# blue-yonder/tsfresh

Hardware: NVIDIA H100
Metric: series/sec extract_features ComprehensiveFCParameters (higher is better)
Workload: dtype f64

## Files before the change

### tsfresh_b200/csrc/k_la.cu

```cuda
#include <algorithm>

#include "tsfx_common.cuh"
#include "tsfx_kernels.h"
#include "tsfx_math.cuh"

namespace tsfx {

__host__ __device__ inline int adf_maxlag(int n) {
    int m = (int)ceil(12.0 * sqrt(sqrt((double)n / 100.0)));
    int cap = n / 2 - 2;
    return m < cap ? m : cap;
}

__device__ __forceinline__ void lag_gram(const double* seq, const double* lev, int t0, int T, int M, double* P, int ldp,
                                         double* C, double* Lv, int lane) {
    for (int d = lane; d <= M; d += 32) {
        double s = 0.0, c = 0.0, l = 0.0;
        for (int t = t0; t < T; ++t) {
            const double v = seq[t - d];
            s = fma(seq[t], v, s);
            c += v;
            if (lev) l = fma(lev[t], v, l);
        }
        C[d] = c;
        if (lev) Lv[d] = l;
        P[d * ldp + 0] = s;
        for (int i = 0; i + 1 + d <= M; ++i) {
            s += seq[t0 - i - 1] * seq[t0 - i - 1 - d] - seq[T - 1 - i] * seq[T - 1 - i - d];
            P[(i + 1 + d) * ldp + (i + 1)] = s;
        }
    }
    __syncwarp();
}

__device__ __forceinline__ int warp_cholesky(double* G, int q, int lda, int lane) {
    for (int j = 0; j < q; ++j) {
        double s = 0.0;
        for (int k = lane; k < j; k += 32) { double v = G[j * lda + k]; s = fma(v, v, s); }
        double d = G[j * lda + j] - wsum(s);
        if (!(d > 0.0)) return j;
        d = sqrt(d);
        __syncwarp();
        if (lane == 0) G[j * lda + j] = d;
        for (int i = j + 1 + lane; i < q; i += 32) {
            double t = G[i * lda + j];
            for (int k = 0; k < j; ++k) t = fma(-G[i * lda + k], G[j * lda + k], t);
            G[i * lda + j] = t / d;
        }
        __syncwarp();
    }
    return q;
}
__device__ __forceinline__ void warp_forward(const double* L, int q, int lda, double* b, int lane) {
    for (int k = 0; k < q; ++k) {
        double zk = b[k] / L[k * lda + k];
        __syncwarp();
        if (lane == 0) b[k] = zk;
        for (int i = k + 1 + lane; i < q; i += 32) b[i] = fma(-L[i * lda + k], zk, b[i]);
        __syncwarp();
    }
}
__device__ __forceinline__ void warp_backward(const double* L, int q, int lda, double* b, int lane) {
    for (int i = q - 1; i >= 0; --i) {
        double xi = b[i] / L[i * lda + i];
        __syncwarp();
        if (lane == 0) b[i] = xi;
        for (int k = lane; k < i; k += 32) b[k] = fma(-L[i * lda + k], xi, b[k]);
        __syncwarp();
    }
}

template <int WPC, bool GS>
__global__ void __launch_bounds__(WPC * 32) k_la(LaArgs A, int pmax) {
    extern __shared__ __align__(16) unsigned char smem_raw[];
    const int lane = threadIdx.x & 31, warp = threadIdx.x >> 5;
    unsigned char* base = warp_region<GS>(smem_raw, A.gscratch, A.bytes_per_warp, WPC, warp);
    double* xc = reinterpret_cast<double*>(base);
    double* dx = xc + A.npad;
    double* G = dx + A.npad;
    double* bvec = G + pmax * pmax;
    double* res = bvec + pmax;
    double* Pm = res + 8;
    double* Cv = Pm + pmax * pmax;
    double* Lv = Cv + pmax;
    float* xs = reinterpret_cast<float*>(Lv + pmax);
    const int64_t warps_total = (int64_t)gridDim.x * WPC;

    for (int64_t s = (int64_t)blockIdx.x * WPC + warp; s < A.R.n_series; s += warps_total) {
        const int n = load_series(A.R, s, xs, lane);
        const Moments M = moments(xs, n, xc, lane);
        for (int i = lane; i + 1 < n; i += 32) dx[i] = (double)xs[i + 1] - (double)xs[i];
        __syncwarp();
        double* orow = A.out + (size_t)s * A.ncols;
        int ar_k = -1; bool ar_ok = false;
        int adf_mode = -1;

        for (int j = 0; j < A.nd; ++j) {
            const Desc d = A.descs[j];
            double r = dnan();
            if (d.calc == TSFX_AR_COEFFICIENT) {
                const int k = d.i1, p = d.i0;
                if (k != ar_k) {
                    ar_k = k;
                    const int rows = n - k;
                    ar_ok = (k < n) && (rows >= k + 1);
                    if (ar_ok) {
                        const int q = k + 1;
                        lag_gram(xc, nullptr, k, n, k, Pm, pmax, Cv, nullptr, lane);
                        for (int e = lane; e < q * q; e += 32) {
                            const int a = e / q, c = e - a * q;
                            if (c > a) continue;
                            G[a * q + c] = (a == 0) ? (double)rows : (c == 0 ? Cv[a] : Pm[a * pmax + c]);
                        }
                        for (int a = lane; a < q; a += 32) bvec[a] = (a == 0) ? Cv[0] : Pm[a * pmax + 0];
                        __syncwarp();
                        int good = 0;
                        if (M.vmax == M.vmin) {
                            double cst = M.vmin, sc = cst / (1.0 + (double)k * cst * cst);
                            for (int a = lane; a < q; a += 32) bvec[a] = (a == 0) ? sc : sc * cst;
                            good = 2;
                        } else if (warp_cholesky(G, q, q, lane) == q) {
                            warp_forward(G, q, q, bvec, lane);
                            warp_backward(G, q, q, bvec, lane);
                            double sphi = 0.0;
                            for (int a = 1 + lane; a < q; a += 32) sphi += bvec[a];
                            sphi = wsum(sphi);
                            if (lane == 0) bvec[0] = bvec[0] + M.mean * (1.0 - sphi);
                            good = 1;
                        }
                        __syncwarp();
                        if (!good) { ar_ok = true; for (int a = lane; a <= k; a += 32) bvec[a] = dnan(); __syncwarp(); }
                    }
                }
                if (p > k) r = dnan();
                else if (!ar_ok) r = (p < k) ? dnan() : 0.0;
                else r = bvec[p];
            } else if (d.calc == TSFX_AUGMENTED_DICKEY_FULLER) {
                if (adf_mode != d.i0) {
                    adf_mode = d.i0;
                    __syncwarp();
                    double stat = dnan(), pval = dnan(), ulag = dnan();
                    const int M0 = adf_maxlag(n);
                    if (M.vmax != M.vmin && M0 >= 0) {
                        const int nd_ = n - 1;
                        int used = M0;
                        if (adf_mode != TSFX_AUTOLAG_NONE) {
                            const int p = M0 + 2, t0 = M0, nobs = nd_ - M0;
                            double* yy = res + 7;
                            lag_gram(dx, xc, t0, nd_, M0, Pm, pmax, Cv, Lv, lane);
                            {
                                double l1 = 0.0, l2 = 0.0;
                                for (int t = t0 + lane; t < nd_; t += 32) { double v = xc[t]; l1 += v; l2 = fma(v, v, l2); }
                                l1 = wsum(l1); l2 = wsum(l2);
                                for (int e = lane; e < p * p; e += 32) {
                                    const int a = e / p, c = e - a * p;
                                    if (c > a) continue;
                                    double v;
                                    if (a == 0) v = (double)nobs;
                                    else if (a == 1) v = (c == 0) ? l1 : l2;
                                    else v = (c == 0) ? Cv[a - 1] : (c == 1 ? Lv[a - 1] : Pm[(a - 1) * pmax + (c - 1)]);
                                    G[a * p + c] = v;
                                }
                                for (int a = lane; a < p; a += 32) bvec[a] = (a == 0) ? Cv[0] : (a == 1 ? Lv[0] : Pm[(a - 1) * pmax + 0]);
                                if (lane == 0) *yy = Pm[0];
                                __syncwarp();
                            }
                            int best_q = 2;
                            {
                                const int okq = warp_cholesky(G, p, p, lane);
                                double ssr = *yy;
                                double ssr_a = 0.0, ssr_b = 0.0;
                                const double dnobs = (double)nobs;
                                for (int i = 0; i < okq; ++i) {
                                    double z = bvec[i] / G[i * p + i];
                                    __syncwarp();
                                    for (int r2 = i + 1 + lane; r2 < okq; r2 += 32) bvec[r2] = fma(-G[r2 * p + i], z, bvec[r2]);
                                    __syncwarp();
                                    ssr -= z * z;
                                    if ((i & 31) == lane) { if (i < 32) ssr_a = ssr; else ssr_b = ssr; }
                                }
                                double ic_a = 0.0, ic_b = 0.0;
#pragma unroll
                                for (int c = 0; c < 2; ++c) {
                                    const int q = c * 32 + lane + 1;
                                    if (q >= 2 && q <= okq) {
                                        const double sq = c ? ssr_b : ssr_a;
                                        const double llf = -dnobs / 2.0 * log(2.0 * 3.14159265358979323846) -
                                                           dnobs / 2.0 * log(sq / dnobs) - dnobs / 2.0;
                                        const double pen = (adf_mode == TSFX_AUTOLAG_AIC) ? 2.0 * (double)q : log(dnobs) * (double)q;
                                        const double ic = -2.0 * llf + pen;
                                        if (c) ic_b = ic; else ic_a = ic;
                                    }
                                }
                                double best_ic = 0.0;
                                bool have = false;
                                for (int q = 2; q <= okq; ++q) {
                                    const double ic = __shfl_sync(FULL, (q > 32) ? ic_b : ic_a, (q - 1) & 31);
                                    if (!have || ic < best_ic) { have = true; best_ic = ic; best_q = q; }
                                }
                            }
                            best_q = __shfl_sync(FULL, best_q, 0);
                            used = best_q - 2;
                            __syncwarp();
                        }
                        const int q = used + 2, t0 = used, nobs = nd_ - used;
                        double* yy = res + 7;
                        lag_gram(dx, xc, t0, nd_, used, Pm, pmax, Cv, Lv, lane);
                        {
                            double l1 = 0.0, l2 = 0.0;
                            for (int t = t0 + lane; t < nd_; t += 32) { double v = xc[t]; l1 += v; l2 = fma(v, v, l2); }
                            l1 = wsum(l1); l2 = wsum(l2);
                            for (int e = lane; e < q * q; e += 32) {
                                const int a = e / q, c = e - a * q;
                                if (c > a) continue;
                                double v;
                                if (a == 0) v = (double)nobs;
                                else if (a < q - 1) v = (c == 0) ? Cv[a] : Pm[a * pmax + c];
                                else v = (c == 0) ? l1 : (c == q - 1 ? l2 : Lv[c]);
                                G[a * q + c] = v;
                            }
                            for (int a = lane; a < q; a += 32) bvec[a] = (a == 0) ? Cv[0] : (a < q - 1 ? Pm[a * pmax + 0] : Lv[0]);
                            if (lane == 0) *yy = Pm[0];
                            __syncwarp();
                        }
                        if (warp_cholesky(G, q, q, lane) == q) {
                            warp_forward(G, q, q, bvec, lane);
                            double ssr = 0.0;
                            for (int i = lane; i < q; i += 32) ssr = fma(bvec[i], bvec[i], ssr);
                            ssr = *yy - wsum(ssr);
                            double s2 = ssr / (double)(nobs - q);
                            stat = bvec[q - 1] / sqrt(s2);
                            pval = m_mackinnon_p_c(stat);
                            ulag = (double)used;
                        }
                        __syncwarp();
                        if (lane == 0) { res[0] = stat; res[1] = pval; res[2] = ulag; }
                    } else if (lane == 0) { res[0] = stat; res[1] = pval; res[2] = ulag; }
                    __syncwarp();
                }
                r = (d.attr >= 0 && d.attr <= 2) ? res[d.attr] : dnan();
            }
            if (lane == 0) orow[d.col] = r;
        }
        __syncwarp();
    }
}

cudaError_t launch_la(const LaArgs& A0, int max_len, cudaStream_t st, int sm_count, const char** variant) {
    static const char* const names[6] = TSFX_GEOM_NAMES("la");
    LaArgs A = A0;
    A.npad = (max_len + 3) & ~3;
    if (adf_maxlag(max_len) + 2 > 64) return cudaErrorInvalidConfiguration;
    int pmax = std::max(adf_maxlag(max_len) + 2, A.nscr + 1);
    pmax = (pmax + 1) & ~1;
    size_t per = (size_t)A.npad * 16 + (size_t)pmax * pmax * 16 + (size_t)pmax * 24 + 64 + (size_t)A.npad * 4;
    per = (per + 15) & ~(size_t)15;
    A.bytes_per_warp = (int)per;
    Geometry G;
    if (!plan_geometry(per, 100 * 1024, 8, A.R.n_series, sm_count, A.gscratch, A.gscratch_bytes, &G)) return cudaErrorInvalidConfiguration;
    A.gscratch = G.gscratch;
    *variant = geom_variant(names, G);
    TSFX_DISPATCH(k_la, G, st, A, pmax)
    return cudaGetLastError();
}

}
```

### tsfresh_b200/csrc/tsfx_api.cu

```cuda
#include <algorithm>
#include <cmath>
#include <cstdio>
#include <cstdlib>
#include <cstring>
#include <condition_variable>
#include <functional>
#include <map>
#include <mutex>
#include <new>
#include <string>
#include <thread>
#include <unordered_map>
#include <vector>

#include "tsfx_common.cuh"
#include "tsfx_kernels.h"
#include "tsfx_csr.h"
#include "tsfx_impute.h"
#include "tsfx_select.h"

using namespace tsfx;

static std::string g_create_error;

// ... 660 lines not shown
            case G_SORTED: {
                SortedArgs A;
                A.R = R; A.gscratch = gs_base; A.gscratch_bytes = slice; A.descs = P->dev[g]; A.nd = (int)P->host[g].size(); A.out = d_out; A.ncols = g_ncols;
                A.nscr = even(4 * (P->friedrich_r + 2) + 16);
                A.nfin = P->sorted_nfin;
                A.ncq = 0;
                {
                    double pl = -1.0, ph = -1.0;
                    for (const Desc& q : P->host[g])
                        if (q.calc == TSFX_CHANGE_QUANTILES && !(q.p0 == pl && q.p1 == ph)) { ++A.ncq; pl = q.p0; ph = q.p1; }
                }
                e = launch_sorted(A, max_len, gs, ctx->sm_count, &variant);
                break;
            }
            case G_SPECTRAL: {
                SpectralArgs A;
                A.R = R; A.gscratch = gs_base; A.gscratch_bytes = slice; A.descs = P->dev[g]; A.nd = (int)P->host[g].size(); A.out = d_out; A.ncols = g_ncols;
                A.twiddle = ctx->d_tw; A.tw_n = ctx->tw_n;
                A.tables = P->d_tables; A.table_off = P->d_toff; A.table_half = P->d_thalf;
                A.need_fft = P->need_fft; A.need_welch = P->need_welch;
                A.max_hist = P->fourier_bins;
                A.nfft = P->spectral_nfft;
                e = launch_spectral(A, max_len, gs, ctx->sm_count, &variant);
                break;
            }
            case G_LA: {
                LaArgs A;
                A.R = R; A.gscratch = gs_base; A.gscratch_bytes = slice; A.descs = P->dev[g]; A.nd = (int)P->host[g].size(); A.out = d_out; A.ncols = g_ncols;
                A.nscr = P->max_ar_k;
                e = launch_la(A, max_len, gs, ctx->sm_count, &variant);
                break;
            }
            case G_ENTROPY: {
                EntropyArgs A;
                A.R = R; A.gscratch = gs_base; A.gscratch_bytes = slice; A.descs = P->dev[g]; A.nd = (int)P->host[g].size(); A.out = d_out; A.ncols = g_ncols;
                e = launch_entropy(A, max_len, gs, ctx->sm_count, &variant);
                break;
            }
            case G_SEQ: {
                SeqArgs A;
                A.R = R; A.gscratch = gs_base; A.gscratch_bytes = slice; A.descs = P->dev[g]; A.nd = (int)P->host[g].size(); A.out = d_out; A.ncols = g_ncols;
                A.nscr = (P->max_lz_bins > 0 ? 1 : 0) | (P->max_perm_dim > 0 ? 2 : 0) | (P->max_cwt_peaks_n << 8) |
                         (std::min(P->n_lz, 255) << 16) | (std::min(P->max_lz_bins, 255) << 24);
                e = launch_seq(A, max_len, gs, ctx->sm_count, &variant);
                break;
            }
            case G_PEAKS: {
                SeqArgs A;
                A.R = R; A.gscratch = gs_base; A.gscratch_bytes = slice; A.descs = P->dev[g]; A.nd = (int)P->host[g].size(); A.out = d_out; A.ncols = g_ncols;
                A.nscr = (P->max_cwt_peaks_n << 8);
                A.ricker = ctx->d_ricker;
                e = launch_peaks(A, max_len, gs, ctx->sm_count, &variant);
                break;
            }
        }
        if (e == cudaErrorInvalidConfiguration) return too_long(kGroupNames[g]);
        if (e != cudaSuccess) return fail(ctx, TSFX_E_CUDA, std::string("launch ") + kGroupNames[g] + ": " + cudaGetErrorString(e));
        ctx->launches += 1;
        ctx->kernels[ctx->n_kernels++] = variant;
        if (timing) { CK(cudaEventRecord(ctx->ev[g][1], ctx->stream)); ctx->ev_used[g] = true; }
    }
    if (nstreams > 1)
        for (int i = 0; i < nstreams - 1; ++i) {
            CK(cudaEventRecord(ctx->ev_join[i], ctx->s_side[i]));
            CK(cudaStreamWaitEvent(ctx->stream, ctx->ev_join[i], 0));
        }
    if (!direct) {
        if (timing) { CK(cudaEventRecord(ctx->ev[G_COUNT][0], ctx->stream)); }
        AssembleArgs A;
        A.stage = (const double*)ctx->stage.p; A.out = d_final; A.n_series = R.n_series; A.ncols = P->ncols; A.ld = ld;
        if (ld != P->ncols && !ctx->peer_out.empty()) return fail(ctx, TSFX_E_UNSUPPORTED, "peer placement of a strided matrix");
        A.n_groups = G_COUNT;
        for (int g = 0; g <= G_COUNT; ++g) A.cum[g] = P->cum[g];
        A.final_col = P->d_final_col;
        A.n_extra = 0;
        A.out_mc = nullptr;
        int64_t peer_off = -1;
        if (!ctx->peer_out.empty()) {
            const uint64_t self = ctx->peer_out[ctx->peer_self];
            if ((uint64_t)d_final < self) return fail(ctx, TSFX_E_INVALID, "out is not inside the matrix registered with tsfx_set_peer_outputs");
            peer_off = (int64_t)((uint64_t)d_final - self);
            if (ctx->peer_mode == TSFX_PEER_MULTICAST) A.out_mc = (double*)(ctx->peer_mc + (uint64_t)peer_off);
            else if (ctx->peer_mode == TSFX_PEER_STORE)
                for (size_t p = 0; p < ctx->peer_out.size(); ++p)
                    if ((int)p != ctx->peer_self) A.extra[A.n_extra++] = (double*)(ctx->peer_out[p] + (uint64_t)peer_off);
        }
        cudaError_t e = launch_assemble(A, ctx->stream, ctx->sm_count);
        if (e != cudaSuccess) return fail(ctx, TSFX_E_CUDA, std::string("launch assemble: ") + cudaGetErrorString(e));
        ctx->launches += 1;
        if (timing) { CK(cudaEventRecord(ctx->ev[G_COUNT][1], ctx->stream)); ctx->ev_used[G_COUNT] = true; }
        if (peer_off >= 0 && ctx->peer_mode == TSFX_PEER_COPY) {
            const size_t bytes = (size_t)R.n_series * P->ncols * sizeof(double);
            CK(cudaEventRecord(ctx->ev_peer, ctx->stream));
            CK(cudaStreamWaitEvent(ctx->s_peer, ctx->ev_peer, 0));
            const size_t np = ctx->peer_out.size();
            for (size_t k = 1; k < np; ++k) {
                const size_t p = ((size_t)ctx->peer_self + k) % np;
                CK(cudaMemcpyAsync((void*)(ctx->peer_out[p] + (uint64_t)peer_off), d_final, bytes, cudaMemcpyDeviceToDevice, ctx->s_peer));
            }
        }
    }
    return TSFX_OK;
}

static int impute_after_extract(tsfx_ctx* ctx, double* d_out, int64_t rows, int cols);
static int nan_error(tsfx_ctx* ctx);

static int check_args(tsfx_ctx* ctx, const tsfx_plan* plan, const void* values, const void* out, int64_t n_series) {
    if (!ctx) return TSFX_E_INVALID;
    if (!plan || plan->ctx != ctx) return fail(ctx, TSFX_E_INVALID, "plan does not belong to this context");
    if (n_series < 0) return fail(ctx, TSFX_E_INVALID, "n_series < 0");
    if (n_series > 0 && (!values || !out)) return fail(ctx, TSFX_E_INVALID, "NULL values/out");
    return TSFX_OK;
}

extern "C" int tsfx_extract_csr(tsfx_ctx* ctx, const tsfx_plan* plan, const float* values, int64_t n_values,
                                const int64_t* begin, const int32_t* len, int64_t n_series, double* out,
                                uint32_t flags) {
    int rc = check_args(ctx, plan, values, out, n_series);
    if (rc) return rc;
    if (n_series == 0) return TSFX_OK;
    if (!begin || !len) return fail(ctx, TSFX_E_INVALID, "NULL begin/len");
    CK(cudaSetDevice(ctx->device));
    SeriesRef R;
    R.dense_len = 0;
    R.n_series = n_series;
    rc = take_times(ctx, plan, n_values, &R.times);
    if (rc) return rc;
    int max_len = 0;
    if (flags & TSFX_FLAG_DEVICE_PTRS) {
        R.values = values; R.begin = begin; R.len = len;
        if (ctx->max_len_hint > 0) max_len = ctx->max_len_hint;
        else {
            int rc2 = csr_max_len(ctx->csr, len, n_series, ctx->stream, &max_len);
            if (rc2) return fail(ctx, TSFX_E_CUDA, "max-length reduction failed");
        }
        rc = run_groups(ctx, plan, R, max_len, out, flags);
        if (!rc && (flags & TSFX_FLAG_IMPUTE)) rc = impute_after_extract(ctx, out, n_series, plan->ncols);
        return rc;
    }
    for (int64_t s = 0; s < n_series; ++s) {
        if (len[s] < 1 || begin[s] < 0 || begin[s] + len[s] > n_values)
            return fail(ctx, TSFX_E_INVALID, "series " + std::to_string(s) + " has an invalid (begin, len)");
        max_len = std::max(max_len, (int)len[s]);
    }
    size_t ob = (size_t)n_series * plan->ncols * sizeof(double);
    CK(ctx->values.reserve((size_t)n_values * sizeof(float) + 16));
    CK(ctx->begin.reserve((size_t)n_series * sizeof(int64_t)));
    CK(ctx->len.reserve((size_t)n_series * sizeof(int32_t)));
    CK(ctx->out.reserve(std::max<size_t>(ob, 8)));
    CK(cudaMemcpyAsync(ctx->values.p, values, (size_t)n_values * sizeof(float), cudaMemcpyHostToDevice, ctx->stream));
    CK(cudaMemcpyAsync(ctx->begin.p, begin, (size_t)n_series * sizeof(int64_t), cudaMemcpyHostToDevice, ctx->stream));
    CK(cudaMemcpyAsync(ctx->len.p, len, (size_t)n_series * sizeof(int32_t), cudaMemcpyHostToDevice, ctx->stream));
    R.values = (const float*)ctx->values.p; R.begin = (const int64_t*)ctx->begin.p; R.len = (const int32_t*)ctx->len.p;
    const bool check_nan = !(flags & TSFX_FLAG_NO_NAN_CHECK);
    if (check_nan) {
        CK(ctx->csr.init_info());
        CK(cudaMemsetAsync(ctx->csr.d_info, 0, sizeof(CsrInfo), ctx->stream));
        csr_check_nan(ctx->csr, R.values, n_values, ctx->stream);
        CK(cudaMemcpyAsync(ctx->csr.h_info, ctx->csr.d_info, sizeof(CsrInfo), cudaMemcpyDeviceToHost, ctx->stream));
    }
    rc = run_groups(ctx, plan, R, max_len, (double*)ctx->out.p, flags);
    if (rc) return rc;
    if (flags & TSFX_FLAG_IMPUTE) { rc = impute_after_extract(ctx, (double*)ctx->out.p, n_series, plan->ncols); if (rc) return rc; }
    CK(cudaMemcpyAsync(out, ctx->out.p, ob, cudaMemcpyDeviceToHost, ctx->stream));
    CK(cudaStreamSynchronize(ctx->stream));
    if (check_nan && ctx->csr.h_info->has_nan) return nan_error(ctx);
    return TSFX_OK;
}

extern "C" int tsfx_extract_dense(tsfx_ctx* ctx, const tsfx_plan* plan, const float* values, int64_t n_series,
                                  int32_t len, double* out, uint32_t flags) {
    int rc = check_args(ctx, plan, values, out, n_series);
    if (rc) return rc;
    if (n_series == 0) return TSFX_OK;
    if (len < 1) return fail(ctx, TSFX_E_INVALID, "len < 1");
    CK(cudaSetDevice(ctx->device));
    SeriesRef R;
    R.begin = nullptr; R.len = nullptr; R.dense_len = len; R.n_series = n_series;
    const int64_t* all_times = nullptr;
    rc = take_times(ctx, plan, n_series * (int64_t)len, &all_times);
    if (rc) return rc;
    R.times = all_times;
    if (flags & TSFX_FLAG_DEVICE_PTRS) {
        R.values = values;
        rc = run_groups(ctx, plan, R, len, out, flags);
        if (!rc && (flags & TSFX_FLAG_IMPUTE)) rc = impute_after_extract(ctx, out, n_series, plan->ncols);
        return rc;
    }
    const size_t ncols = (size_t)plan->ncols;
    const size_t vb = (size_t)n_series * len * sizeof(float), ob = (size_t)n_series * ncols * sizeof(double);
    CK(ctx->values.reserve(vb + 16));
    CK(ctx->out.reserve(std::max<size_t>(ob, 8)));
    int64_t block = std::max<int64_t>(16384, (n_series + 15) / 16);
    if (flags & TSFX_FLAG_TIMING) block = n_series;
    float* dv = (float*)ctx->values.p;
    double* dout = (double*)ctx->out.p;
    const bool check_nan = !(flags & TSFX_FLAG_NO_NAN_CHECK);
    if (check_nan) { CK(ctx->csr.init_info()); CK(cudaMemsetAsync(ctx->csr.d_info, 0, sizeof(CsrInfo), ctx->stream)); }
    int nb = 0;
    for (int64_t lo = 0; lo < n_series; lo += block, ++nb) {
        const int64_t cnt = std::min<int64_t>(block, n_series - lo);
        const int slot = nb & 1;
        CK(ctx->stager.h2d(dv + (size_t)lo * len, values + (size_t)lo * len, (size_t)cnt * len * sizeof(float), ctx->s_in));
        CK(cudaEventRecord(ctx->ev_in[slot], ctx->s_in));
        CK(cudaStreamWaitEvent(ctx->stream, ctx->ev_in[slot], 0));
        if (check_nan) csr_check_nan(ctx->csr, dv + (size_t)lo * len, cnt * len, ctx->stream);
        R.values = dv + (size_t)lo * len;
        R.times = all_times ? all_times + (size_t)lo * len : nullptr;
        R.n_series = cnt;
        rc = run_groups(ctx, plan, R, len, dout + (size_t)lo * ncols, flags);
        if (rc) return rc;
        if (flags & TSFX_FLAG_IMPUTE) continue;
        CK(cudaEventRecord(ctx->ev_done[slot], ctx->stream));
        CK(cudaStreamWaitEvent(ctx->s_out, ctx->ev_done[slot], 0));
        CK(cudaMemcpyAsync(out + (size_t)lo * ncols, dout + (size_t)lo * ncols, (size_t)cnt * ncols * sizeof(double),
                           cudaMemcpyDeviceToHost, ctx->s_out));
    }
    if (flags & TSFX_FLAG_IMPUTE) {
        rc = impute_after_extract(ctx, dout, n_series, plan->ncols);
        if (rc) return rc;
        CK(cudaMemcpyAsync(out, dout, ob, cudaMemcpyDeviceToHost, ctx->stream));
    }
    if (check_nan) CK(cudaMemcpyAsync(ctx->csr.h_info, ctx->csr.d_info, sizeof(CsrInfo), cudaMemcpyDeviceToHost, ctx->stream));
    CK(cudaStreamSynchronize(ctx->s_out));
    CK(cudaStreamSynchronize(ctx->stream));
    if (check_nan && ctx->csr.h_info->has_nan) return nan_error(ctx);
    return TSFX_OK;
}

static int impute_after_extract(tsfx_ctx* ctx, double* d_out, int64_t rows, int cols) {
    int n = 0;
    cudaError_t e = impute_device(ctx->imp, d_out, rows, cols, TSFX_IMPUTE_RANGE, false, nullptr, ctx->sm_count, ctx->stream, &n);
    if (e != cudaSuccess) return fail(ctx, TSFX_E_CUDA, std::string("impute: ") + cudaGetErrorString(e));
    ctx->launches += n;
    return TSFX_OK;
}

extern "C" int tsfx_impute(tsfx_ctx* ctx, double* matrix, int64_t n_rows, int32_t n_cols, int32_t mode, double* col_stats,
                           uint32_t flags) {
    if (!ctx) return TSFX_E_INVALID;
    if (n_rows < 0 || n_cols < 0 || mode < TSFX_IMPUTE_RANGE || mode > TSFX_IMPUTE_STATS)
        return fail(ctx, TSFX_E_INVALID, "tsfx_impute: bad arguments");
    if (n_rows == 0 || n_cols == 0) return TSFX_OK;
    if (!matrix) return fail(ctx, TSFX_E_INVALID, "tsfx_impute: NULL matrix");
    if ((mode == TSFX_IMPUTE_GIVEN || mode == TSFX_IMPUTE_STATS) && !col_stats)
        return fail(ctx, TSFX_E_INVALID, "tsfx_impute: col_stats is required for this mode");
    if (mode == TSFX_IMPUTE_GIVEN)
        for (int64_t i = 0; i < (int64_t)3 * n_cols; ++i)
            if (!std::isfinite(col_stats[i]))
                return fail(ctx, TSFX_E_INVALID, "tsfx_impute: non-finite replacement value");
    CK(cudaSetDevice(ctx->device));
    const size_t bytes = (size_t)n_rows * n_cols * sizeof(double);
    double* d_m = matrix;
    const bool host = !(flags & TSFX_FLAG_DEVICE_PTRS);
    if (host) {
        CK(ctx->out.reserve(bytes));
        d_m = (double*)ctx->out.p;
        CK(cudaMemcpyAsync(d_m, matrix, bytes, cudaMemcpyHostToDevice, ctx->stream));
    }
    int n = 0;
    cudaError_t e = impute_device(ctx->imp, d_m, n_rows, n_cols, mode, (flags & TSFX_FLAG_ALL_MEDIANS) != 0 || mode == TSFX_IMPUTE_STATS,
                                  col_stats, ctx->sm_count, ctx->stream, &n);
    if (e != cudaSuccess) return fail(ctx, TSFX_E_CUDA, std::string("impute: ") + cudaGetErrorString(e));
    ctx->launches = n;
    if (host) {
        if (mode != TSFX_IMPUTE_STATS) CK(cudaMemcpyAsync(matrix, d_m, bytes, cudaMemcpyDeviceToHost, ctx->stream));
        CK(cudaStreamSynchronize(ctx->stream));
    }
    return TSFX_OK;
}

extern "C" int tsfx_get_timings(tsfx_ctx* ctx, float* ms_out, const char** names_out, int32_t cap) {
    if (!ctx) return TSFX_E_INVALID;
    CK(cudaSetDevice(ctx->device));
    CK(cudaStreamSynchronize(ctx->stream));
    int k = 0;
    for (int g = 0; g < G_EVENTS && k < cap; ++g) {
        if (!ctx->ev_used[g]) continue;
        float ms = 0.f;
        CK(cudaEventElapsedTime(&ms, ctx->ev[g][0], ctx->ev[g][1]));
        if (ms_out) ms_out[k] = ms;
        if (names_out) names_out[k] = (g == G_BASIC && ctx->used_moments) ? "moments" : kGroupNames[g];
        ++k;
    }
    return k;
}

extern "C" int tsfx_last_launch_count(const tsfx_ctx* ctx) { return ctx ? ctx->launches : 0; }

extern "C" int tsfx_last_kernels(const tsfx_ctx* ctx, const char** names_out, int32_t cap) {
    if (!ctx || cap < 0 || (cap > 0 && !names_out)) return TSFX_E_INVALID;
    const int k = std::min<int>(ctx->n_kernels, cap);
    for (int i = 0; i < k; ++i) names_out[i] = ctx->kernels[i];
    return k;
}

#define TSFX_GEOM_LIST(GRP) GRP "/w8/shared", GRP "/w4/shared", GRP "/w2/shared", GRP "/w1/shared", GRP "/w4/global", GRP "/w1/global"
static const char* const kKernelVariants[] = {
    "moments/dense", "moments/general",
    "basic/w12/shared", "basic/w24/shared", TSFX_GEOM_LIST("basic"),
    "sorted/w12/shared", TSFX_GEOM_LIST("sorted"),
    TSFX_GEOM_LIST("spectral"), TSFX_GEOM_LIST("spectral/pow2"),
    TSFX_GEOM_LIST("la"),
    "entropy/rank-g1", "entropy/rank-g4", "entropy/rank-g16", TSFX_GEOM_LIST("entropy/tiles"), TSFX_GEOM_LIST("entropy/pairs"),
    "seq/small", TSFX_GEOM_LIST("seq/general"),
    "peaks/small", TSFX_GEOM_LIST("peaks/general"), "peaks/general/hybrid/w4/global", "peaks/general/hybrid/w1/global",
};
#undef TSFX_GEOM_LIST

extern "C" int tsfx_kernel_variants(const char** names_out, int32_t cap) {
    const int n = (int)(sizeof(kKernelVariants) / sizeof(kKernelVariants[0]));
    for (int i = 0; i < n && i < cap && names_out; ++i) names_out[i] = kKernelVariants[i];
    return n;
}

struct LongIn {
    const int64_t* ids;
    const void* keys;
    int is_f64;
    const float* values;
    int64_t n;
    bool device;
    const float* const* more = nullptr;
    int n_kinds = 1;
    const float* col(int k) const { return k == 0 ? values : more[k - 1]; }
};

static inline size_t kind_stride(int64_t n) { return ((size_t)n + 3) & ~(size_t)3; }

static int nan_error(tsfx_ctx* ctx) { return fail(ctx, TSFX_E_NAN, "the value column contains NaN"); }

static int stage_a(tsfx_ctx* ctx, const LongIn& in, int max_blocks, bool check_nan, CsrInfo* info, bool* streamed,
                   const int64_t** d_ids_out, const uint64_t** d_keys_out, const float** d_vals_out) {
    CsrWorkspace& W = ctx->csr;
    std::string msg;
    const int64_t n = in.n;
    const int64_t* d_ids = in.ids;
    const uint64_t* d_keys = (const uint64_t*)in.keys;
    const float* d_vals = in.values;
    if (!in.device) {
        CK(W.reserve(0, (size_t)n * 8));
        CK(W.reserve(2, (size_t)n * 4 + 16));
        if (in.keys) CK(W.reserve(1, (size_t)n * 8));
        CK(ctx->stager.h2d(W.ids(), in.ids, (size_t)n * 8, ctx->stream));
        d_ids = W.ids();
        d_keys = in.keys ? W.keys() : nullptr;
        d_vals = W.vals();
    }
    int rc = csr_ids_pass(W, d_ids, n, 16384, max_blocks, ctx->stream, &msg);
    if (rc) return fail(ctx, rc, msg);
    CK(cudaStreamSynchronize(ctx->stream));
    *info = *W.h_info;
    *streamed = false;
    if (!info->unsorted_ids) {
        W.d_values = const_cast<float*>(d_vals);
        if (!in.device) *streamed = true;
        else csr_check_rows(W, d_ids, d_keys, in.is_f64, d_vals, 0, n, check_nan, ctx->stream);
    }
    *d_ids_out = d_ids; *d_keys_out = d_keys; *d_vals_out = d_vals;
    return TSFX_OK;
}

static int stage_a_sort(tsfx_ctx* ctx, const LongIn& in, int max_blocks, bool check_nan, CsrInfo* info,
                        const int64_t* d_ids, const uint64_t* d_keys, const float* d_vals) {
    CsrWorkspace& W = ctx->csr;
    std::string msg;
    if (!in.device) {
        if (in.keys) CK(ctx->stager.h2d(W.keys(), in.keys, (size_t)in.n * 8, ctx->stream));
        CK(ctx->stager.h2d(W.vals(), in.values, (size_t)in.n * 4, ctx->stream));
    }
    int rc = csr_sort_pass(W, d_ids, d_keys, in.is_f64, d_vals, in.n, 16384, max_blocks, check_nan, ctx->stream, &msg);
    if (rc) return fail(ctx, rc, msg);
    CK(cudaStreamSynchronize(ctx->stream));
    *info = *W.h_info;
    return TSFX_OK;
}

extern "C" int tsfx_build_csr(tsfx_ctx* ctx, const int64_t* ids, const void* sort_keys, int32_t sort_key_is_f64,
                              const float* values, int64_t n_rows, int64_t* out_ids, int64_t* out_begin,
                              int32_t* out_len, float* sorted_values, int64_t out_capacity, int64_t* n_series_out) {
    if (!ctx) return TSFX_E_INVALID;
    if (n_rows < 0 || !n_series_out || (n_rows > 0 && (!ids || !values)))
        return fail(ctx, TSFX_E_INVALID, "tsfx_build_csr: bad arguments");
    CK(cudaSetDevice(ctx->device));
    *n_series_out = 0;
    if (n_rows == 0) return TSFX_OK;
    ctx->held_series = -1;
    LongIn in{ids, sort_keys, sort_key_is_f64, values, n_rows, false};
    CsrInfo info;
    bool streamed = false;
    const int64_t* d_ids; const uint64_t* d_keys; const float* d_vals;
    int rc = stage_a(ctx, in, 1, true, &info, &streamed, &d_ids, &d_keys, &d_vals);
    if (rc) return rc;
    CsrWorkspace& W = ctx->csr;
    bool need_sort = info.unsorted_ids != 0;
    if (!need_sort) {
        if (sort_keys) CK(ctx->stager.h2d(W.keys(), sort_keys, (size_t)n_rows * 8, ctx->stream));
        CK(ctx->stager.h2d(W.vals(), values, (size_t)n_rows * 4, ctx->stream));
        csr_check_rows(W, d_ids, d_keys, sort_key_is_f64, d_vals, 0, n_rows, true, ctx->stream);
        CK(cudaMemcpyAsync(W.h_info, W.d_info, sizeof(CsrInfo), cudaMemcpyDeviceToHost, ctx->stream));
        CK(cudaStreamSynchronize(ctx->stream));
        info = *W.h_info;
        need_sort = info.unsorted_keys != 0;
        if (need_sort) {
            LongIn dev{d_ids, d_keys, sort_key_is_f64, d_vals, n_rows, true};
            rc = stage_a_sort(ctx, dev, 1, true, &info, d_ids, d_keys, d_vals);
            if (rc) return rc;
        }
    } else {
        rc = stage_a_sort(ctx, in, 1, true, &info, d_ids, d_keys, d_vals);
        if (rc) return rc;
    }
    if (info.has_nan) return nan_error(ctx);
    const int64_t ns = info.n_series;
    ctx->held_series = ns;
    ctx->held_max_len = info.max_len;
    *n_series_out = ns;
    if (!out_ids && !out_begin && !out_len && !sorted_values) return TSFX_OK;
    if (ns > out_capacity) return fail(ctx, TSFX_E_INVALID, "out_capacity too small: " + std::to_string(ns) + " series");
    if (out_ids) CK(cudaMemcpyAsync(out_ids, W.d_uid, ns * sizeof(int64_t), cudaMemcpyDeviceToHost, ctx->stream));
    if (out_begin) CK(cudaMemcpyAsync(out_begin, W.d_begin, ns * sizeof(int64_t), cudaMemcpyDeviceToHost, ctx->stream));
    if (out_len) CK(cudaMemcpyAsync(out_len, W.d_len, ns * sizeof(int32_t), cudaMemcpyDeviceToHost, ctx->stream));
    if (sorted_values) CK(cudaMemcpyAsync(sorted_values, W.d_values, n_rows * sizeof(float), cudaMemcpyDeviceToHost, ctx->stream));
    CK(cudaStreamSynchronize(ctx->stream));
    return TSFX_OK;
}

#define TSFX_MAX_KINDS 64
struct KindSet {
    int n = 1;
    const tsfx_plan* plan[TSFX_MAX_KINDS];
    const float* dvals[TSFX_MAX_KINDS];
    int col0[TSFX_MAX_KINDS];
    int total_cols = 0;
};

static int run_blocks(tsfx_ctx* ctx, const KindSet& K, const CsrInfo& info, const LongIn* stream_in,
                      const int64_t* d_ids, const uint64_t* d_keys, bool check_rows, bool check_nan,
                      double* out, bool out_is_device, uint32_t flags, const int64_t* row_times = nullptr) {
    CsrWorkspace& W = ctx->csr;
    const size_t ncols = (size_t)K.total_cols;
    const int64_t ns = info.n_series;
    double* dout = out;
    if (!out_is_device) {
        CK(ctx->out.reserve(std::max<size_t>((size_t)ns * ncols * sizeof(double), 8)));
        dout = (double*)ctx->out.p;
    }
    const bool impute = (flags & TSFX_FLAG_IMPUTE) != 0;
    for (int b = 0; b < info.n_blocks; ++b) {
        const int64_t s0 = info.series_lo[b], s1 = info.series_lo[b + 1];
        const int64_t r0 = info.row_lo[b], r1 = info.row_lo[b + 1];
        const int slot = b & 1;
        if (stream_in) {
            if (stream_in->keys) CK(ctx->stager.h2d(W.keys() + r0, (const uint64_t*)stream_in->keys + r0, (size_t)(r1 - r0) * 8, ctx->s_in));
            for (int k = 0; k < K.n; ++k)
                CK(ctx->stager.h2d(const_cast<float*>(K.dvals[k]) + r0, stream_in->col(k) + r0, (size_t)(r1 - r0) * 4, ctx->s_in));
            CK(cudaEventRecord(ctx->ev_in[slot], ctx->s_in));
            CK(cudaStreamWaitEvent(ctx->stream, ctx->ev_in[slot], 0));
        }
        if (check_rows) {
            csr_check_rows(W, d_ids, d_keys, stream_in ? stream_in->is_f64 : 0, K.dvals[0], r0, r1, check_nan, ctx->stream);
            if (check_nan) for (int k = 1; k < K.n; ++k) csr_check_nan(W, K.dvals[k] + r0, r1 - r0, ctx->stream);
        }
        for (int k = 0; k < K.n; ++k) {
            if (K.plan[k]->ncols == 0) continue;
            SeriesRef R;
            R.values = K.dvals[k]; R.begin = W.d_begin + s0; R.len = W.d_len + s0; R.dense_len = 0; R.n_series = s1 - s0;
            R.times = row_times;
            int rc = run_groups(ctx, K.plan[k], R, info.max_len, dout + (size_t)s0 * ncols + K.col0[k], flags, K.total_cols);
            if (rc) return rc;
        }
        if (impute || out_is_device) continue;
        CK(cudaEventRecord(ctx->ev_done[slot], ctx->stream));
        CK(cudaStreamWaitEvent(ctx->s_out, ctx->ev_done[slot], 0));
        CK(cudaMemcpyAsync(out + (size_t)s0 * ncols, dout + (size_t)s0 * ncols, (size_t)(s1 - s0) * ncols * sizeof(double),
                           cudaMemcpyDeviceToHost, ctx->s_out));
    }
    if (impute) {
        int rc = impute_after_extract(ctx, dout, ns, K.total_cols);
        if (rc) return rc;
        if (!out_is_device) CK(cudaMemcpyAsync(out, dout, (size_t)ns * ncols * sizeof(double), cudaMemcpyDeviceToHost, ctx->stream));
    }
    return TSFX_OK;
}

static int extract_long_impl(tsfx_ctx* ctx, const tsfx_plan* const* plans, const LongIn& in, int64_t* out_ids, double* out,
                             int64_t out_capacity, int64_t** out_ids_alloc, double** out_alloc, int64_t* n_series_out,
                             uint32_t flags) {
    CsrWorkspace& W = ctx->csr;
    const tsfx_plan* plan = plans[0];
    KindSet K;
    K.n = in.n_kinds;
    if (K.n < 1 || K.n > TSFX_MAX_KINDS) return fail(ctx, TSFX_E_INVALID, "between 1 and 64 kinds per call");
    for (int k = 0; k < K.n; ++k) {
        if (!plans[k] || plans[k]->ctx != ctx) return fail(ctx, TSFX_E_INVALID, "plan does not belong to this context");
        K.plan[k] = plans[k];
        K.col0[k] = K.total_cols;
        K.total_cols += plans[k]->ncols;
    }
    for (int k = 0; k < K.n; ++k) if (plans[k]->need_times) plan = plans[k];
    const size_t kstride = kind_stride(in.n);
    if (K.n > 1 && !in.device) CK(ctx->kvals.reserve((size_t)(K.n - 1) * kstride * 4 + 16));
    const bool check_nan = !(flags & TSFX_FLAG_NO_NAN_CHECK);
    const int max_blocks = (flags & TSFX_FLAG_TIMING) ? 1 : 16;
    ctx->held_series = -1;
    const int64_t* times_in = nullptr;
    int rc = take_times(ctx, plan, in.n, &times_in);
    if (rc) return rc;
    CsrInfo info;
    bool streamed = false;
    const int64_t* d_ids; const uint64_t* d_keys; const float* d_vals;
    rc = stage_a(ctx, in, max_blocks, check_nan, &info, &streamed, &d_ids, &d_keys, &d_vals);
    if (rc) return rc;
    bool sorted = !info.unsorted_ids;
    bool extra_resident = in.device;
    auto extra_in = [&](int k) -> const float* {
        return in.device ? in.col(k) : (const float*)ctx->kvals.p + (size_t)(k - 1) * kstride;
    };
    if (sorted && in.device && check_nan)
        for (int k = 1; k < K.n; ++k) csr_check_nan(W, in.col(k), in.n, ctx->stream);
    for (int attempt = 0; attempt < 2; ++attempt) {
        if (!sorted) {
            rc = stage_a_sort(ctx, in, max_blocks, check_nan, &info, d_ids, d_keys, d_vals);
            if (rc) return rc;
            if (info.has_nan) return nan_error(ctx);
        }
        K.dvals[0] = W.d_values;
        if (K.n > 1) {
            if (W.d_perm) {
                CK(ctx->kvals_sorted.reserve((size_t)(K.n - 1) * kstride * 4 + 16));
                for (int k = 1; k < K.n; ++k) {
                    if (!extra_resident) CK(ctx->stager.h2d(const_cast<float*>(extra_in(k)), in.col(k), (size_t)in.n * 4, ctx->stream));
                    if (check_nan) csr_check_nan(W, extra_in(k), in.n, ctx->stream);
                    float* dst = (float*)ctx->kvals_sorted.p + (size_t)(k - 1) * kstride;
                    csr_gather_f32(W, extra_in(k), dst, in.n, ctx->stream);
                    K.dvals[k] = dst;
                }
                extra_resident = true;
            } else {
                for (int k = 1; k < K.n; ++k) K.dvals[k] = extra_in(k);
            }
        }
        const int64_t ns = info.n_series;
        *n_series_out = ns;
        const size_t ob = (size_t)ns * K.total_cols * sizeof(double);
        if (out_alloc) {
            if (!*out_alloc) {
                *out_alloc = (double*)ctx->pool.alloc(std::max<size_t>(ob, 8));
                *out_ids_alloc = (int64_t*)ctx->pool.alloc(std::max<size_t>((size_t)ns * 8, 8));
                if (!*out_alloc || !*out_ids_alloc) return fail(ctx, TSFX_E_NOMEM, "pinned host allocation failed");
            }
            out = *out_alloc;
            out_ids = *out_ids_alloc;
        } else if (ns > out_capacity) {
            return fail(ctx, TSFX_E_INVALID, "out_capacity too small: " + std::to_string(ns) + " series");
        }
        if (info.max_len < 1 && ns > 0) return fail(ctx, TSFX_E_INVALID, "empty series");
        const bool first_sorted_try = sorted && attempt == 0;
        const int64_t* row_times = times_in;
        if (times_in && W.d_perm) {
            CK(ctx->times_sorted.reserve((size_t)in.n * 8));
            csr_gather_i64(W, times_in, (int64_t*)ctx->times_sorted.p, in.n, ctx->stream);
            row_times = (const int64_t*)ctx->times_sorted.p;
        }
        rc = run_blocks(ctx, K, info, (first_sorted_try && streamed) ? &in : nullptr, d_ids, d_keys,
                        first_sorted_try && streamed, check_nan, out, in.device, flags, row_times);
        if (first_sorted_try && streamed) extra_resident = true;
        if (rc) return rc;
        if (out_ids) CK(cudaMemcpyAsync(out_ids, W.d_uid, (size_t)ns * sizeof(int64_t), in.device ? cudaMemcpyDeviceToDevice : cudaMemcpyDeviceToHost, ctx->stream));
        if (in.device && !first_sorted_try) break;
        const bool late_nan_flags = !first_sorted_try && K.n > 1 && check_nan;
        if (first_sorted_try || late_nan_flags) CK(cudaMemcpyAsync(W.h_info, W.d_info, sizeof(CsrInfo), cudaMemcpyDeviceToHost, ctx->stream));
        CK(cudaStreamSynchronize(ctx->s_out));
        CK(cudaStreamSynchronize(ctx->stream));
        if (late_nan_flags && W.h_info->has_nan) return nan_error(ctx);
        if (!first_sorted_try) break;
        if (W.h_info->has_nan) return nan_error(ctx);
        if (!W.h_info->unsorted_keys) break;
        sorted = false;
        if (!in.device) {
            LongIn dev{d_ids, d_keys, in.is_f64, d_vals, in.n, true};
            rc = stage_a_sort(ctx, dev, max_blocks, check_nan, &info, d_ids, d_keys, d_vals);
            if (rc) return rc;
            if (info.has_nan) return nan_error(ctx);
            sorted = true;
            streamed = false;
        }
    }
    ctx->held_series = info.n_series;
    ctx->held_max_len = info.max_len;
    return TSFX_OK;
}

extern "C" int tsfx_extract_long(tsfx_ctx* ctx, const tsfx_plan* plan, const int64_t* ids, const void* sort_keys,
                                 int32_t sort_key_is_f64, const float* values, int64_t n_rows, int64_t* out_ids,
                                 double* out, int64_t out_capacity, int64_t* n_series_out, uint32_t flags) {
    if (!ctx) return TSFX_E_INVALID;
    if (!plan || plan->ctx != ctx) return fail(ctx, TSFX_E_INVALID, "plan does not belong to this context");
    const bool reuse = (ids == nullptr && values == nullptr);
    if (n_rows < 0 || !n_series_out || (!reuse && n_rows > 0 && (!ids || !values)) || !out)
        return fail(ctx, TSFX_E_INVALID, "tsfx_extract_long: bad arguments");
    CK(cudaSetDevice(ctx->device));
    *n_series_out = 0;
    if (reuse) {
        if (flags & TSFX_FLAG_DEVICE_PTRS) return fail(ctx, TSFX_E_INVALID, "the held CSR is extracted into host buffers");
        if (ctx->held_series < 0) return fail(ctx, TSFX_E_INVALID, "tsfx_extract_long: no CSR is held by this context");
// ... 214 lines not shown
```

Measured before the change: 4.456 million.

## Add register-resident small-series linear-algebra kernel for AR and ADF features

Adds a specialized k_la_small kernel for series up to 256 points with few AR lags. Gram matrices are built with a warp reduce-scatter plus incremental edge corrections, and Cholesky factorization runs with rows held in registers using a refined approximate rsqrt. ADF lag selection reuses a single full factorization to derive SSR for every lag. This is meant to cut the shared/global scratch traffic and per-lag refactorization of the generic path, at the cost of more register pressure and subtle numeric differences.

```diff
diff --git a/tsfresh_b200/csrc/k_la.cu b/tsfresh_b200/csrc/k_la.cu
--- a/tsfresh_b200/csrc/k_la.cu
+++ b/tsfresh_b200/csrc/k_la.cu
@@ -246,8 +246,344 @@
     }
 }
 
+#define LA_SMALL_LEN 256
+#define LA_SMALL_KMAX 15
+#define LA_SMALL_P 19
+#define LA_SMALL_LD 19
+#define LA_SMALL_WPC 8
+#define LA_SMALL_CB (LA_SMALL_P + 64)
+
+__device__ __forceinline__ double rsqrt_pos(double d) {
+    double y;
+    asm("rsqrt.approx.ftz.f64 %0, %1;" : "=d"(y) : "d"(d));
+#pragma unroll
+    for (int it = 0; it < 2; ++it) y = fma(0.5 * y, fma(-d * y, y, 1.0), y);
+    return y;
+}
+
+template <int O>
+__device__ __forceinline__ void reduce_scatter_stage(double (&v)[32], int lane) {
+    const bool up = lane & O;
+#pragma unroll
+    for (int i = 0; i < O; ++i) {
+        const double lo = v[i], hi = v[i + O];
+        const double send = up ? lo : hi;
+        const double keep = up ? hi : lo;
+        v[i] = keep + __shfl_xor_sync(FULL, send, O);
+    }
+    if constexpr (O > 1) reduce_scatter_stage<O / 2>(v, lane);
+}
+__device__ __forceinline__ double reduce_scatter32(double (&v)[32], int lane) {
+    reduce_scatter_stage<16>(v, lane);
+    return v[0];
+}
+
+__device__ __forceinline__ double pick(const double (&g)[LA_SMALL_P], int i) {
+    double r = 0.0;
+#pragma unroll
+    for (int c = 0; c < LA_SMALL_P; ++c)
+        if (c == i) r = g[c];
+    return r;
+}
+
+__device__ __forceinline__ int chol_rows(double (&g)[LA_SMALL_P], int na, int nf, double& inv, double* cb, int lane) {
+    double* piv = cb;
+    int done = nf;
+    if (lane == 0) piv[0] = g[0];
+#pragma unroll
+    for (int j = 0; j < LA_SMALL_P - 1; ++j) {
+        if (j < done) {
+            __syncwarp();
+            const double d = piv[j];
+            if (!(d > 0.0)) {
+                done = j;
+            } else {
+                double* col = cb + LA_SMALL_P + 32 * (j & 1);
+                const double rinv = rsqrt_pos(d), r = d * rinv;
+                const double l = (lane == j) ? r : g[j] * rinv;
+                if (lane == j) inv = rinv;
+                if (lane >= j) g[j] = l;
+                col[lane] = l;
+                __syncwarp();
+#pragma unroll
+                for (int c = j + 1; c < LA_SMALL_P; ++c) {
+                    const double lc = col[c];
+                    g[c] = (lane > j) ? fma(-l, lc, g[c]) : (lane == j ? lc : g[c]);
+                }
+                if (j + 1 < LA_SMALL_P && lane == j + 1) piv[j + 1] = g[j + 1];
+            }
+        }
+    }
+    __syncwarp();
+    return done;
+}
+
+template <typename F>
+__device__ __forceinline__ void load_rows(double (&g)[LA_SMALL_P], const double* Gs, int na, F col, int lane) {
+    const double* row = Gs + (lane < na ? col(lane) : 0) * LA_SMALL_LD;
+#pragma unroll
+    for (int c = 0; c < LA_SMALL_P; ++c) g[c] = (c < na && lane < na) ? row[col(c)] : 0.0;
+}
+
+template <int NL>
+__device__ __forceinline__ void ar_sums(double (&v)[32], const double* xs, int n, int k, double mean, int lane) {
+#pragma unroll 1
+    for (int t = k + lane; t < n; t += 32) {
+        const double w = xs[t] - mean;
+        v[16] += w;
+#pragma unroll
+        for (int d = 0; d < NL; ++d) v[d] = fma(w, xs[max(t - d, 0)] - mean, v[d]);
+    }
+}
+
+__device__ __forceinline__ void ar_gram(const double* xs, int n, int k, double mean, double* Gs, int lane) {
+    double v[32];
+#pragma unroll
+    for (int i = 0; i < 32; ++i) v[i] = 0.0;
+    if (k <= 10) ar_sums<11>(v, xs, n, k, mean, lane);
+    else ar_sums<LA_SMALL_KMAX + 1>(v, xs, n, k, mean, lane);
+    const double tot = reduce_scatter32(v, lane);
+    const double c0 = __shfl_sync(FULL, tot, 16);
+    __syncwarp();
+    const int q = k + 1;
+    auto col = [&](int i) { return i == 0 ? q : i; };
+    auto xc = [&](int i) { return xs[i] - mean; };
+    if (lane <= k) {
+        const int d = lane;
+        double s = tot, c = c0;
+        Gs[col(d) * LA_SMALL_LD + col(0)] = s;
+        Gs[col(0) * LA_SMALL_LD + col(d)] = s;
+        for (int m = 0; m + 1 + d <= k; ++m) {
+            s += xc(k - m - 1) * xc(k - m - 1 - d) - xc(n - 1 - m) * xc(n - 1 - m - d);
+            Gs[col(m + 1 + d) * LA_SMALL_LD + col(m + 1)] = s;
+            Gs[col(m + 1) * LA_SMALL_LD + col(m + 1 + d)] = s;
+        }
+        for (int m = 0; m < d; ++m) c += xc(k - 1 - m) - xc(n - 1 - m);
+        Gs[col(d)] = c;
+        Gs[col(d) * LA_SMALL_LD] = c;
+    }
+    if (lane == 0) Gs[0] = (double)(n - k);
+    __syncwarp();
+}
+
+__device__ __forceinline__ void adf_gram(const double* xs, int n, int M0, double mean, double* Gs, int lane) {
+    const int nd = n - 1, t0 = M0, p = M0 + 2;
+    auto xd = [&](int i) { return xs[i]; };
+    auto dx = [&](int i) { return xd(i + 1) - xd(i); };
+    auto col = [&](int i) { return i == 0 ? p : i + 1; };
+    double sums[2];
+#pragma unroll
+    for (int pass = 0; pass < 2; ++pass) {
+        double v[32];
+#pragma unroll
+        for (int i = 0; i < 32; ++i) v[i] = 0.0;
+#pragma unroll 1
+        for (int t = t0 + lane; t < nd; t += 32) {
+            double hi = xd(t + 1), lo = xd(t);
+            const double y = hi - lo, lev = lo - mean;
+            const double w = pass ? lev : y;
+            if (!pass) { v[17] += lev; v[18] = fma(lev, lev, v[18]); }
+#pragma unroll
+            for (int d = 0; d <= 16; ++d) {
+                if (d > 0) { hi = lo; lo = xd(max(t - d, 0)); }
+                v[d] = fma(w, hi - lo, v[d]);
+            }
+        }
+        sums[pass] = reduce_scatter32(v, lane);
+    }
+    const double tot = sums[0], lv = sums[1];
+    const double l1 = __shfl_sync(FULL, tot, 17), l2 = __shfl_sync(FULL, tot, 18);
+    __syncwarp();
+    if (lane <= M0) {
+        const int d = lane;
+        double s = tot;
+        Gs[col(d) * LA_SMALL_LD + col(0)] = s;
+        Gs[col(0) * LA_SMALL_LD + col(d)] = s;
+        for (int m = 0; m + 1 + d <= M0; ++m) {
+            s += dx(t0 - m - 1) * dx(t0 - m - 1 - d) - dx(nd - 1 - m) * dx(nd - 1 - m - d);
+            Gs[col(m + 1 + d) * LA_SMALL_LD + col(m + 1)] = s;
+            Gs[col(m + 1) * LA_SMALL_LD + col(m + 1 + d)] = s;
+        }
+        const double c = xd(nd - d) - xd(t0 - d);
+        Gs[col(d)] = c;
+        Gs[col(d) * LA_SMALL_LD] = c;
+        Gs[LA_SMALL_LD + col(d)] = lv;
+        Gs[col(d) * LA_SMALL_LD + 1] = lv;
+    }
+    if (lane == 0) {
+        Gs[0] = (double)(nd - M0);
+        Gs[1] = Gs[LA_SMALL_LD] = l1;
+        Gs[LA_SMALL_LD + 1] = l2;
+    }
+    __syncwarp();
+}
+
+template <int WPC, int MINB>
+__global__ void __launch_bounds__(WPC * 32, MINB) k_la_small(LaArgs A) {
+    extern __shared__ __align__(16) unsigned char smem_raw[];
+    const int lane = threadIdx.x & 31, warp = threadIdx.x >> 5;
+    unsigned char* base = smem_raw + (size_t)warp * A.bytes_per_warp;
+    double* xs = reinterpret_cast<double*>(base);
+    double* Gs = xs + LA_SMALL_LEN;
+    double* cb = Gs + LA_SMALL_P * LA_SMALL_LD;
+    double* arb = cb + LA_SMALL_CB;
+
+    for (int64_t s = (int64_t)blockIdx.x * WPC + warp; s < A.R.n_series; s += (int64_t)gridDim.x * WPC) {
+        float* stage = reinterpret_cast<float*>(Gs);
+        const int n = load_series(A.R, s, stage, lane);
+        const Moments M = moments(stage, n, nullptr, lane);
+        for (int i = lane; i < n; i += 32) xs[i] = (double)stage[i];
+        __syncwarp();
+        const bool flat = M.vmax == M.vmin;
+        int ar_k = -1; bool ar_ok = false;
+        int adf_mode = -1; bool adf_gram_ok = false;
+
+        for (int j = 0; j < A.nd; ++j) {
+            const Desc d = A.descs[j];
+            double r = dnan();
+            if (d.calc == TSFX_AR_COEFFICIENT) {
+                const int k = d.i1, p = d.i0;
+                if (k != ar_k) {
+                    ar_k = k;
+                    const int rows = n - k;
+                    ar_ok = (k < n) && (rows >= k + 1);
+                    if (ar_ok) {
+                        const int q = k + 1;
+                        if (flat) {
+                            const double cst = M.vmin, sc = cst / (1.0 + (double)k * cst * cst);
+                            if (lane < q) arb[lane] = (lane == 0) ? sc : sc * cst;
+                        } else {
+                            ar_gram(xs, n, k, M.mean, Gs, lane);
+                            adf_gram_ok = false;
+                            double g[LA_SMALL_P], inv = 0.0;
+                            load_rows(g, Gs, q + 1, [](int i) { return i; }, lane);
+                            if (chol_rows(g, q + 1, q, inv, cb, lane) == q) {
+                                double b = pick(g, q);
+#pragma unroll
+                                for (int i = LA_SMALL_P - 2; i >= 0; --i) {
+                                    if (i < q) {
+                                        if (lane == i) arb[i] = b * inv;
+                                        __syncwarp();
+                                        if (lane < i) b = fma(-g[i], arb[i], b);
+                                    }
+                                }
+                                if (lane == 0) {
+                                    double sphi = 0.0;
+                                    for (int a = 1; a < q; ++a) sphi += arb[a];
+                                    arb[0] = arb[0] + M.mean * (1.0 - sphi);
+                                }
+                            } else if (lane < q) {
+                                arb[lane] = dnan();
+                            }
+                        }
+                        __syncwarp();
+                    }
+                }
+                if (p > k) r = dnan();
+                else if (!ar_ok) r = (p < k) ? dnan() : 0.0;
+                else r = arb[p];
+            } else if (d.calc == TSFX_AUGMENTED_DICKEY_FULLER) {
+                if (adf_mode != d.i0) {
+                    adf_mode = d.i0;
+                    double stat = dnan(), pval = dnan(), ulag = dnan();
+                    const int M0 = adf_maxlag(n);
+                    if (!flat && M0 >= 0) {
+                        const int nd_ = n - 1, p = M0 + 2;
+                        if (!adf_gram_ok) { adf_gram(xs, n, M0, M.mean, Gs, lane); adf_gram_ok = true; }
+                        int used = M0;
+                        if (adf_mode != TSFX_AUTOLAG_NONE) {
+                            double g[LA_SMALL_P], inv = 0.0;
+                            load_rows(g, Gs, p + 1, [](int i) { return i; }, lane);
+                            const int okq = chol_rows(g, p + 1, p, inv, cb, lane);
+                            if (lane == p) {
+#pragma unroll
+                                for (int c = 0; c < LA_SMALL_P - 1; ++c) cb[c] = g[c];
+                            }
+                            __syncwarp();
+                            const double dnobs = (double)(nd_ - M0);
+                            double ssr = Gs[p * LA_SMALL_LD + p], ssr_q = 0.0;
+                            for (int i = 0; i < okq; ++i) {
+                                const double z = cb[i];
+                                ssr -= z * z;
+                                if (lane == i) ssr_q = ssr;
+                            }
+                            double ic = 0.0;
+                            const int q = lane + 1;
+                            if (q >= 2 && q <= okq) {
+                                const double llf = -dnobs / 2.0 * log(2.0 * 3.14159265358979323846) -
+                                                   dnobs / 2.0 * log(ssr_q / dnobs) - dnobs / 2.0;
+                                const double pen = (adf_mode == TSFX_AUTOLAG_AIC) ? 2.0 * (double)q : log(dnobs) * (double)q;
+                                ic = -2.0 * llf + pen;
+                            }
+                            __syncwarp();
+                            cb[lane] = ic;
+                            __syncwarp();
+                            int best_q = 2;
+                            double best_ic = 0.0;
+                            bool have = false;
+                            for (int qq = 2; qq <= okq; ++qq) {
+                                const double icq = cb[qq - 1];
+                                if (!have || icq < best_ic) { have = true; best_ic = icq; best_q = qq; }
+                            }
+                            __syncwarp();
+                            used = best_q - 2;
+                        }
+                        const int q = used + 2, na = q + 1;
+                        auto fcol = [&](int f) { return f == 0 ? 0 : f <= used ? f + 1 : f == used + 1 ? 1 : p; };
+                        double g[LA_SMALL_P], inv = 0.0;
+                        load_rows(g, Gs, na, fcol, lane);
+                        for (int t = used; t < M0; ++t) {
+                            double v = 0.0;
+                            if (lane == 0) v = 1.0;
+                            else if (lane <= used) v = xs[t - lane + 1] - xs[t - lane];
+                            else if (lane == used + 1) v = xs[t] - M.mean;
+                            else if (lane == used + 2) v = xs[t + 1] - xs[t];
+                            cb[lane] = v;
+                            __syncwarp();
+#pragma unroll
+                            for (int c = 0; c < LA_SMALL_P; ++c)
+                                if (c < na) g[c] = fma(v, cb[c], g[c]);
+                            __syncwarp();
+                        }
+                        if (chol_rows(g, na, q, inv, cb, lane) == q) {
+                            if (lane == q) { cb[0] = pick(g, q - 1); cb[1] = pick(g, q); }
+                            __syncwarp();
+                            const double z = cb[0], ssr = cb[1];
+                            const double s2 = ssr / (double)(nd_ - used - q);
+                            stat = z / sqrt(s2);
+                            pval = m_mackinnon_p_c(stat);
+                            ulag = (double)used;
+                        }
+                    }
+                    __syncwarp();
+                    if (lane == 0) { arb[16] = stat; arb[17] = pval; arb[18] = ulag; }
+                    __syncwarp();
+                }
+                r = (d.attr >= 0 && d.attr <= 2) ? arb[16 + d.attr] : dnan();
+            }
+            if (lane == 0) A.out[(size_t)s * A.ncols + d.col] = r;
+        }
+        __syncwarp();
+    }
+}
+
 cudaError_t launch_la(const LaArgs& A0, int max_len, cudaStream_t st, int sm_count, const char** variant) {
     static const char* const names[6] = TSFX_GEOM_NAMES("la");
+    if (max_len <= LA_SMALL_LEN && A0.nscr <= LA_SMALL_KMAX) {
+        LaArgs A = A0;
+        A.npad = LA_SMALL_LEN;
+        A.bytes_per_warp = (LA_SMALL_LEN + LA_SMALL_P * LA_SMALL_LD + LA_SMALL_CB + 32) * 8;
+        A.gscratch = nullptr;
+        const size_t smem = (size_t)A.bytes_per_warp * LA_SMALL_WPC;
+        const int64_t ctas = (A.R.n_series + LA_SMALL_WPC - 1) / LA_SMALL_WPC;
+        const int64_t cap = (int64_t)sm_count * grid_waves(4096);
+        const int grid = (int)std::max<int64_t>(1, std::min(ctas, cap));
+        *variant = "la/small";
+        cudaError_t e = cudaFuncSetAttribute(k_la_small<LA_SMALL_WPC, 3>, cudaFuncAttributeMaxDynamicSharedMemorySize, (int)smem);
+        if (e != cudaSuccess) return e;
+        k_la_small<LA_SMALL_WPC, 3><<<grid, LA_SMALL_WPC * 32, smem, st>>>(A);
+        return cudaGetLastError();
+    }
     LaArgs A = A0;
     A.npad = (max_len + 3) & ~3;
     if (adf_maxlag(max_len) + 2 > 64) return cudaErrorInvalidConfiguration;
diff --git a/tsfresh_b200/csrc/tsfx_api.cu b/tsfresh_b200/csrc/tsfx_api.cu
--- a/tsfresh_b200/csrc/tsfx_api.cu
+++ b/tsfresh_b200/csrc/tsfx_api.cu
@@ -986,7 +986,7 @@
     "basic/w12/shared", "basic/w24/shared", TSFX_GEOM_LIST("basic"),
     "sorted/w12/shared", TSFX_GEOM_LIST("sorted"),
     TSFX_GEOM_LIST("spectral"), TSFX_GEOM_LIST("spectral/pow2"),
-    TSFX_GEOM_LIST("la"),
+    "la/small", TSFX_GEOM_LIST("la"),
     "entropy/rank-g1", "entropy/rank-g4", "entropy/rank-g16", TSFX_GEOM_LIST("entropy/tiles"), TSFX_GEOM_LIST("entropy/pairs"),
     "seq/small", TSFX_GEOM_LIST("seq/general"),
     "peaks/small", TSFX_GEOM_LIST("peaks/general"), "peaks/general/hybrid/w4/global", "peaks/general/hybrid/w1/global",
```

New measurement: 4.689 million (median of 6 runs). 1.05x the previous value.
